# moddyz/stereo-to-multiview-cuda

Measured on AMD Instinct MI355X. Metric: stereo->8-view frames/sec @1080p d=64; cost-agg HBM GB/s vs roofline, higher is better.
Workload: dtype f32; 1 GPU; 1920x1080 synthetic stereo frame, D=64, zd=32, full stereo->8-view frame: cost init + cross aggregation + WTA + DCC/IRV x5/bilateral + 6 DIBR views + interlacing, one frame per GPU per step; stages=3, usd=34, lsd=17, views=8, aggregation=matrix pipe (stm_kernels_aggm.hip)

## Files before the change

stereo-to-multiview-cuda_amd/csrc/stm_common.h:

```cpp
#pragma once
#include <hip/hip_runtime.h>
#include <stddef.h>
#include <stdint.h>

typedef unsigned char u8;

namespace stm {

void fail(const char *what, const char *expr, const char *file, int line);
bool failed();
void clear_failed();
struct ApiNest { ApiNest(); ~ApiNest(); };
bool api_outermost();
void release_host_frame_bufs();
bool nv12_args_ok(const char *fn, int num_rows, int num_cols_sbs, int num_cols, const char *cols_name, int pitch_y, int pitch_uv, int matrix);
#define STM_CHECK(expr)                                                                  \
    do {                                                                                 \
        hipError_t _e = (expr);                                                          \
        if (_e != hipSuccess) ::stm::fail(hipGetErrorString(_e), #expr, __FILE__, __LINE__); \
    } while (0)
#define STM_CHECK_LAUNCH() STM_CHECK(hipGetLastError())
#define STM_LAUNCH(...)                                     \
    do {                                                    \
        if (!::stm::failed()) hipLaunchKernelGGL(__VA_ARGS__); \
// ... 314 lines not shown
bool balance_params_ok(const char *fn, int mode, const u8 *lut768);
bool balance_auto_params_ok(const char *fn, int max_shift, float rate);
bool balance_size_ok(const char *fn, int num_rows, int num_cols);
int balance_rate_q(float rate);
constexpr size_t BALANCE_HIST_WORDS = 1536, BALANCE_STATE_WORDS = 769;
void launch_balance_measure(int *state, uint32_t *hist, const PackInput *in, const u8 *img_l, const u8 *img_r, int H, int W, int elem_sz,
                            int max_shift, int rate_q, bool fresh);
void launch_balance_frame(u8 *out, const PackInput *in, const u8 *img, int H, int W, int elem_sz, const u8 *lut768, const int *state);
struct Cut {
    int mode;
    int thresh_permille, min_gap;
    int *d_state;
};
Cut cut_default();
Cut cut();
void set_cut(const Cut &c);
bool cut_params_ok(const char *fn, int thresh_permille, int min_gap);
bool cut_size_ok(const char *fn, int num_rows, int num_cols);
constexpr size_t CUT_SIG_WORDS = 256, CUT_STATE_WORDS = 260;
constexpr int CUT_DEFAULT_THRESH = 370;
void launch_cut_detect(int *state, uint32_t *sig, const PackInput *in, const u8 *img_l, int H, int W, int elem_sz, int thresh_permille,
                       int min_gap, void *reset0, void *reset1, void *reset2);
struct Active {
    int mode;
    int rect[4];
    int fill;
    float fill_disp;
    int thresh_luma, lit_permille, max_bar_permille, hold;
    int *d_state;
};
Active active_default();
Active active();
void set_active(const Active &a);
bool active_params_ok(const char *fn, int mode, const int *rect, int fill, float fill_disp);
bool active_auto_params_ok(const char *fn, int thresh_luma, int lit_permille, int max_bar_permille, int hold);
bool active_size_ok(const char *fn, int num_rows, int num_cols);
bool active_rect_ok(const char *fn, const int *rect, int num_rows, int num_cols);
constexpr size_t ACTIVE_STATE_WORDS = 16;
void launch_active_detect(int *state, uint32_t *counts, const PackInput *in, const u8 *img_l, int H, int W, int elem_sz, int thresh_luma,
                          int lit_permille, int max_bar_permille, int hold, bool restart, const int *cut_state);
void launch_active_rect(int *d_rect, const int rect[4]);
void launch_active_fill(int nmaps, float *const *disp, int H, int W, const int *d_rect, float value);
struct AggTap {
    float *h1, *v2, *h4;
    const float *inject_v2;
    bool on() const { return h1 || v2 || h4 || inject_v2; }
};
AggTap agg_tap();
void set_agg_tap(const AggTap &t);
enum { TAP_PQ = 0, TAP_PX = 1, TAP_QUADS = 2 };
void launch_tap_read(const float *vol_l, const float *vol_r, int layout, int ord, float *dst, int D, int H, int W);
void launch_tap_write(float *vol_l, float *vol_r, int layout, int ord, const float *src, int D, int H, int W);
struct PQViews {
    const uint32_t *pk[2], *cen[2];
    float *a[2], *b[2];
    const u8 *armU[2], *armD[2], *armL[2], *armR[2];
    float *disp[2];
};
size_t pq_volume_floats(int D, int H, int W);
bool aggm_supports(int usd, int H, int W);
void launch_aggm_frame(const uint32_t *const *pk, const uint32_t *const *cen, const float *lut, float *const *vol_a, float *const *vol_b,
                       const u8 *const *armU, const u8 *const *armD, const u8 *const *armL, const u8 *const *armR, float *const *disp,
                       int D, int zd, int H, int W, int usd, bool keep_volume = false, uint32_t *htab_ready = nullptr, uint32_t *vtab_ready = nullptr,
                       bool v2_read_later = false);
size_t aggm_frame_htab_dwords(int D, int H, int W, int usd, bool keep_volume);
size_t aggm_frame_vtab_dwords(int D, int zd, int H, int W, int usd, bool keep_volume, bool v2_read_later, int *rec, int *top, bool *col);
bool aggm_frame_px(int D, int zd, int H, int W, int usd, bool keep_volume, bool v2_read_later);
int aggm_frame_px_order(int D, int zd, int H, int W, int usd, bool keep_volume, bool v2_read_later);
int aggm_frame_path(int D, int zd, int H, int W, int usd, bool keep_volume, bool v2_read_later);
int aggm_frame_hc2_parts(int D, int zd, int H, int W, int usd, bool keep_volume, bool v2_read_later);
bool launch_aggm_stage(Vol in, Vol out, const u8 *armU, const u8 *armD, const u8 *armL, const u8 *armR, int D, int H, int W, int usd);
size_t aggm_stage_bytes(int D, int H, int W, int usd);
bool aggh_supports(int usd, int D);
size_t aggh_table_dwords(int nviews, int H, int W);
void launch_hwin_table(PQViews &v, int nviews, uint32_t *tab, int H, int W);
void launch_pq_hsr(PQViews &v, int nviews, const uint32_t *tab, int D, int zd, int H, int W, bool px = false, int ord = 0);
bool aggv_supports(int usd);
int aggv_table_top();
int aggv_table_rec();
void launch_pq_v12q(PQViews &v, int nviews, const uint32_t *tab, int rec, int H, int W, int G, int NC);
void launch_pq_v12r(PQViews &v, int nviews, const uint32_t *tab, int H, int W, int G, bool x4 = false);
void launch_vcol_table(PQViews &v, int nviews, uint32_t *tab, int H, int W);
size_t aggv_col_table_dwords(int nviews, int H, int W);
void launch_to_pq(Vol in, float *pq, int D, int H, int W, uint32_t *odd = nullptr);
void launch_from_pq(const float *pq, Vol out, int D, int H, int W);
void launch_hslo_wta(int nviews, const Vol *cost, const u8 *const *img_a, const u8 *const *img_b, const int *osign,
                     float *const *disp, float T, float H1, float H2, int D, int zd, int H, int W, int elem_sz);
void launch_hslo_wta_pq(int nviews, float *const *cost_pq, float *const *acc_pq, const u8 *const *img_a, const u8 *const *img_b,
                        const int *osign, float *const *disp, float T, float H1, float H2, int D, int zd, int H, int W, int elem_sz);

void rho_luts(float ad_coeff, float census_coeff, float *lut_ad , float *lut_census );
void gaussian_kernel_2d(float *kernel, int radius, float sigma);
void gaussian_kernel_1d(float *kernel, int size, float sigma);
float mux_y_interval(int num_views, float angle, int elem_sz);

}
```

stereo-to-multiview-cuda_amd/csrc/stm_hwin.h:

```cpp
#pragma once
#include "stm_common.h"

namespace stm {

constexpr int HR_TOP = 36;
constexpr int HR_NG = 22;
constexpr int HR_REC = 64;

template <int N> __device__ __forceinline__ int hr_row_ror(int v) { return __builtin_amdgcn_update_dpp(0, v, 0x120 + N, 0xf, 0xf, false); }

template <int N> __device__ __forceinline__ uint32_t hr_row_shr(uint32_t v) { return (uint32_t)__builtin_amdgcn_update_dpp(0, (int)v, 0x110 + N, 0xf, 0xf, false); }

static __device__ __forceinline__ void win16_build(uint32_t *__restrict__ dst, uint32_t *ev, int R0, int s0, int nn)
{
    const int m = threadIdx.x & 15;
    int lo = nn ? s0 : 0x7fffffff, hi = nn ? s0 + nn : -0x7fffffff;
    lo = min(lo, hr_row_ror<8>(lo)); lo = min(lo, hr_row_ror<4>(lo)); lo = min(lo, hr_row_ror<2>(lo)); lo = min(lo, hr_row_ror<1>(lo));
    hi = max(hi, hr_row_ror<8>(hi)); hi = max(hi, hr_row_ror<4>(hi)); hi = max(hi, hr_row_ror<2>(hi)); hi = max(hi, hr_row_ror<1>(hi));
    const int K0 = hi > lo ? (lo & ~3) : 0, n = hi > lo ? (hi - K0 + 3) >> 2 : 0;
    const int q0 = n ? (K0 - R0) >> 2 : 0;
#pragma unroll
    for (int i = 0; i < 6; ++i) ev[6 * m + i] = 0u;
    __builtin_amdgcn_wave_barrier();
    if (nn) {
        atomicXor(&ev[s0 - K0], 1u << m);
        atomicXor(&ev[s0 + nn - K0], 1u << m);
    }
    __builtin_amdgcn_wave_barrier();
    uint32_t e[6];
#pragma unroll
    for (int i = 0; i < 6; ++i) e[i] = ev[6 * m + i];
#pragma unroll
    for (int i = 1; i < 6; ++i) e[i] ^= e[i - 1];
    uint32_t tot = e[5];
    tot ^= hr_row_shr<1>(tot); tot ^= hr_row_shr<2>(tot); tot ^= hr_row_shr<4>(tot); tot ^= hr_row_shr<8>(tot);
    const uint32_t before = hr_row_shr<1>(tot);
    __builtin_amdgcn_wave_barrier();
#pragma unroll
    for (int i = 0; i < 6; ++i) ev[6 * m + i] = e[i] ^ before;
    __builtin_amdgcn_wave_barrier();
    if (!dst) return;
    if (m < 2) dst[m] = m == 0 ? (uint32_t)q0 : (uint32_t)n;
#pragma unroll
    for (int j = m; j < HR_NG; j += 16)
        if (j < n) {
            const unsigned long long mk = (unsigned long long)ev[4 * j] | ((unsigned long long)ev[4 * j + 1] << 16) |
                                          ((unsigned long long)ev[4 * j + 2] << 32) | ((unsigned long long)ev[4 * j + 3] << 48);
            *(unsigned long long *)(dst + 8 + 2 * (HR_NG - n + j)) = mk;
        }
}

static __device__ __forceinline__ void hwin_build(uint32_t *__restrict__ tab, uint32_t *ev4, int y, int x0, int aL, int aR, int W, int nTx)
{
    const int l = threadIdx.x & 63, r = l >> 4;
    const int x = x0 + l, t = x >> 4;
    int s0 = 0, nn = 0;
    if (x < W) {
        s0 = x - aL;
        nn = aL + aR;
    }
    win16_build(t < nTx ? tab + ((size_t)y * nTx + t) * HR_REC : nullptr, ev4 + r * 96, 16 * t - HR_TOP, s0, nn);
}

static __device__ __forceinline__ void vcol_build(uint32_t *__restrict__ tile, uint32_t *ev4, int u, int x0, int s0, int nn)
{
    const int r = (threadIdx.x & 63) >> 4;
    win16_build(tile + (size_t)(x0 + r) * HR_REC, ev4 + r * 96, 16 * u - HR_TOP, s0, nn);
}

__device__ __forceinline__ int hw_wave_min_i(int v)
{
    v = min(v, hr_row_ror<8>(v)); v = min(v, hr_row_ror<4>(v)); v = min(v, hr_row_ror<2>(v)); v = min(v, hr_row_ror<1>(v));
    return min(min(__builtin_amdgcn_readlane(v, 0), __builtin_amdgcn_readlane(v, 16)),
               min(__builtin_amdgcn_readlane(v, 32), __builtin_amdgcn_readlane(v, 48)));
}
__device__ __forceinline__ int hw_wave_max_i(int v)
{
    v = max(v, hr_row_ror<8>(v)); v = max(v, hr_row_ror<4>(v)); v = max(v, hr_row_ror<2>(v)); v = max(v, hr_row_ror<1>(v));
    return max(max(__builtin_amdgcn_readlane(v, 0), __builtin_amdgcn_readlane(v, 16)),
               max(__builtin_amdgcn_readlane(v, 32), __builtin_amdgcn_readlane(v, 48)));
}
static __device__ __forceinline__ void vwin_build(uint32_t *__restrict__ dst, unsigned long long *ev, int u, int top, int s0, int nn)
{
    const int l = threadIdx.x & 63;
    const int lo = hw_wave_min_i(nn ? s0 : 0x7fffffff);
    const int hi = hw_wave_max_i(nn ? s0 + nn : -0x7fffffff);
    const int K0 = hi > lo ? (lo & ~3) : 0, n_it = hi > lo ? (hi - K0 + 3) >> 2 : 0;
    const int q0 = top >= 0 && n_it ? (K0 - (16 * u - top)) >> 2 : 0;
    if (l < 8) dst[l] = l == 0 ? (uint32_t)(top >= 0 ? q0 : K0) : l == 1 ? (uint32_t)n_it : 0u;
    unsigned long long *mk = (unsigned long long *)(dst + 8) + 4 * q0;
    const int steps = 4 * n_it;
    for (int j = l; j <= steps; j += 64) ev[j] = 0ull;
    __builtin_amdgcn_wave_barrier();
    if (nn) {
        atomicXor(&ev[s0 - K0], 1ull << l);
        atomicXor(&ev[s0 + nn - K0], 1ull << l);
    }
    __builtin_amdgcn_wave_barrier();
    unsigned long long carry = 0ull;
    for (int base = 0; base < steps; base += 64) {
        unsigned long long e = base + l < steps ? ev[base + l] : 0ull;
#pragma unroll
        for (int o = 1; o < 64; o <<= 1) {
            const unsigned long long t = __shfl_up(e, o);
            if (l >= o) e ^= t;
        }
        e ^= carry;
        if (base + l < steps) mk[base + l] = e;
        carry = __shfl(e, 63);
    }
}

}
```

stereo-to-multiview-cuda_amd/csrc/stm_kernels_agg.hip:

```cpp
#include "stm_hwin.h"

namespace stm {

constexpr uint32_t W10_ONE = 1u | (1u << 10) | (1u << 20);
constexpr uint32_t W10_GUARD = 512u * W10_ONE;

__global__ __launch_bounds__(256) void stm_k_widen_px(const uint32_t *__restrict__ bgrx, uint32_t *__restrict__ wide, int n)
{
    const int i = blockIdx.x * 256 + threadIdx.x;
    if (i >= n) return;
    const uint32_t p = bgrx[i];
    wide[i] = (p & 0xffu) | ((p & 0xff00u) << 2) | ((p & 0xff0000u) << 4);
}


struct ArmsArgs {
    const uint32_t *img[2];
    u8 *up[2], *down[2], *left[2], *right[2];
    uint32_t *htab;
    uint32_t *vtab;
    int vrec, vtop;
    int vcol;
};

// ... 106 lines not shown
        _Pragma("unroll") for (int d = 0; d < 4; ++d)                                                                   \
        {                                                                                                               \
            CT[d] = C[d] + tg_near;                                                                                     \
            const uint32_t ok = (CT[d] - anchor) & (anchor_n - C[d]) & (CT[d] - P[d]) & (PT[d] - C[d]) & W10_GUARD;     \
            STM_ARM_VERDICT(d, ok == W10_GUARD)                                                                         \
        }                                                                                                               \
    }
#define STM_ARM_FAR(K)                                                                     \
    {                                                                                      \
        uint32_t c[4];                                                                     \
        STM_ARM_LOADS(c, K)                                                                \
        _Pragma("unroll") for (int d = 0; d < 4; ++d)                                      \
        {                                                                                  \
            const uint32_t ok = (c[d] + far_lo) & (far_hi - c[d]) & W10_GUARD;             \
            STM_ARM_VERDICT(d, ok == W10_GUARD)                                            \
        }                                                                                  \
    }
    const uint32_t anchor_n = anchor + tg_near;
    uint32_t ca[4], ta[4], cb[4] = {anchor, anchor, anchor, anchor}, tb[4] = {anchor_n, anchor_n, anchor_n, anchor_n};
    const int knear = max(0, min(usd, lsd));
#define STM_ARM_ANY_OPEN (((open[0] | open[1]) | (open[2] | open[3])) != 0ull)
    for (int k = 1; k < knear; k += 2) {
        STM_ARM_CLOSE(k)
        STM_ARM_NEAR(k, ca, ta, cb, tb)
        STM_ARM_NEAR(k + 1, cb, tb, ca, ta)
    }
    if ((knear & 1) && STM_ARM_ANY_OPEN) STM_ARM_NEAR(knear, ca, ta, cb, tb)
    const uint32_t far_lo = tg_far - anchor, far_hi = anchor + tg_far;
    for (int k = knear + 1; k < usd; k += 2) {
        STM_ARM_CLOSE(k)
        STM_ARM_FAR(k)
        STM_ARM_FAR(k + 1)
    }
    if (usd > knear && ((usd - knear) & 1) && STM_ARM_ANY_OPEN) STM_ARM_FAR(usd)
#undef STM_ARM_ANY_OPEN
#undef STM_ARM_FAR
#undef STM_ARM_NEAR
#undef STM_ARM_CLOSE
#undef STM_ARM_VERDICT
#undef STM_ARM_LOADS
    arm[0] = min(arm[0], kmaxU);
    arm[1] = min(arm[1], kmaxD);
    arm[2] = min(arm[2], kmaxL);
    arm[3] = min(arm[3], kmaxR);
}
template <int MODE, bool VMIN>
static __device__ __forceinline__ void cross_arms_body(const ArmsArgs &a, uint32_t tg_far, uint32_t tg_near, int usd, int lsd, int H, int W)
{
    constexpr bool HTAB = MODE >= 1;
    const int v = blockIdx.z;
    const int wv_ = __builtin_amdgcn_readfirstlane((int)(threadIdx.x >> 6));
    const int xr = MODE == 2 ? blockIdx.x * 64 + (threadIdx.x & 63) : blockIdx.x * 256 + threadIdx.x;
    const int yr = MODE == 2 ? blockIdx.y * 16 + wv_ : blockIdx.y;
    if (MODE == 1 ? (xr & ~63) >= W : MODE == 0 ? xr >= W : false) return;
    const int x = min(xr, W - 1), y = min(yr, H - 1);
    const int p = y * W + x;
    int arm[4];
    if (VMIN) cross_arms_walk_vmin(a.img[v], x, y, p, tg_far, tg_near, usd, lsd, H, W, arm);
    else cross_arms_walk(a.img[v], x, y, tg_far, tg_near, usd, lsd, H, W, arm);
    const bool inside = xr < W && yr < H;
    if (inside) {
        a.up[v][p] = (u8)arm[0];
        a.down[v][p] = (u8)arm[1];
        a.left[v][p] = (u8)arm[2];
        a.right[v][p] = (u8)arm[3];
    }
    __shared__ uint32_t ev_all[MODE == 2 ? 16 : 4][4 * 96];
    if (HTAB) {
        const int nTx = (W + 15) >> 4;
        if (yr < H)
            hwin_build(a.htab + (size_t)v * H * nTx * HR_REC, ev_all[wv_], yr, xr & ~63, arm[2], arm[3], W, nTx);
    }
    if (MODE == 2) {
        __shared__ u8 s_u[16][64], s_d[16][64];
        __shared__ unsigned long long ev_v[16][96];
        const int l = threadIdx.x & 63;
        s_u[wv_][l] = inside ? (u8)arm[0] : (u8)0;
        s_d[wv_][l] = inside ? (u8)arm[1] : (u8)0;
        __syncthreads();
        const int G = (W + 3) >> 2, nT = (H + 15) >> 4, gg = blockIdx.x * 16 + wv_, u = blockIdx.y;
        if (gg < G) {
            const int b = l >> 4, i = l & 15;
            const int aU = s_u[i][4 * wv_ + b], aD = s_d[i][4 * wv_ + b];
            if (a.vcol)
                vcol_build(a.vtab + (size_t)(v * nT + u) * (4 * G) * HR_REC, ev_all[wv_], u, 4 * gg, blockIdx.y * 16 + i - aU, aU + aD);
            else
                vwin_build(a.vtab + ((size_t)(v * nT + u) * G + gg) * a.vrec, ev_v[wv_], u, a.vtop, blockIdx.y * 16 + i - aU, aU + aD);
        }
    }
}

template <int MODE>
__global__ __launch_bounds__(MODE == 2 ? 1024 : 256) void stm_k_cross_arms(ArmsArgs a, uint32_t tg_far, uint32_t tg_near, int usd, int lsd, int H, int W)
{
    cross_arms_body<MODE, false>(a, tg_far, tg_near, usd, lsd, H, W);
}

template <int MODE>
__global__ __launch_bounds__(MODE == 2 ? 1024 : 256) void stm_k_cross_arms_vmin(ArmsArgs a, uint32_t tg_far, uint32_t tg_near, int usd, int lsd, int H, int W)
{
    cross_arms_body<MODE, true>(a, tg_far, tg_near, usd, lsd, H, W);
}

static uint32_t wide_threshold(float t)
{
    int ti;
    if (t != t) ti = 255;
    else if (t >= 255.f) ti = 255;
    else if (t < 0.f) ti = -1;
    else ti = (int)floorf(t);
    return (uint32_t)(512 + ti) * W10_ONE;
}

void launch_cross_arms2(int nviews, const uint32_t *const *packed, u8 *const *up, u8 *const *down, u8 *const *left,
                        u8 *const *right, float ucd, float lcd, int usd, int lsd, int H, int W, const uint32_t *const *wide_ready,
                        uint32_t *htab, uint32_t *vtab, int vrec, int vtop, bool vcol)
{
    ArmsArgs a;
    const int n = H * W;
    ProfScope p("cross_arms");
    const uint32_t *wide[2];
    for (int v = 0; v < nviews; ++v) {
        if (wide_ready) {
            wide[v] = wide_ready[v];
            continue;
        }
        uint32_t *w = Workspace::get<uint32_t>((size_t)n);
        STM_LAUNCH(stm_k_widen_px, dim3(cdiv(n, 256)), dim3(256), 0, stream(), packed[v], w, n);
        STM_CHECK_LAUNCH();
        wide[v] = w;
    }
    for (int v = 0; v < 2; ++v) {
        const int s = v < nviews ? v : 0;
        a.img[v] = wide[s]; a.up[v] = up[s]; a.down[v] = down[s]; a.left[v] = left[s]; a.right[v] = right[s];
    }
    if (usd > 255) usd = 255;
    a.htab = htab;
    a.vtab = vtab;
    a.vrec = vrec;
    a.vtop = vtop;
    a.vcol = vcol ? 1 : 0;
    const bool vmin = (agg_variant() / 100) % 10 == 7 || (size_t)H * W * 4 >= ((size_t)1 << 31);
    const uint32_t tg_far = wide_threshold(ucd), tg_near = wide_threshold(lcd);
#define STM_CROSS_LAUNCH(MODE, GRID, BLOCK)                                                                                      \
    {                                                                                                                            \
        if (vmin) STM_LAUNCH(stm_k_cross_arms_vmin<MODE>, GRID, BLOCK, 0, stream(), a, tg_far, tg_near, usd, lsd, H, W);         \
        else STM_LAUNCH(stm_k_cross_arms<MODE>, GRID, BLOCK, 0, stream(), a, tg_far, tg_near, usd, lsd, H, W);                   \
    }
    if (htab && vtab && vtop >= 0 && usd <= HR_TOP && usd <= vtop)
        STM_CROSS_LAUNCH(2, dim3(cdiv(W, 64), cdiv(H, 16), nviews), dim3(1024))
    else if (htab && usd <= HR_TOP)
        STM_CROSS_LAUNCH(1, dim3(cdiv(W, 256), H, nviews), dim3(256))
    else
        STM_CROSS_LAUNCH(0, dim3(cdiv(W, 256), H, nviews), dim3(256))
#undef STM_CROSS_LAUNCH
    STM_CHECK_LAUNCH();
}

void launch_cross_arms(const uint32_t *packed, u8 *up, u8 *down, u8 *left, u8 *right, float ucd, float lcd, int usd,
                       int lsd, int H, int W)
{
    launch_cross_arms2(1, &packed, &up, &down, &left, &right, ucd, lcd, usd, lsd, H, W, nullptr);
}

#define STM_ACC(s, v) { s.x = s.x + v.x; s.y = s.y + v.y; s.z = s.z + v.z; s.w = s.w + v.w; }

template <int S> __device__ __forceinline__ float4 window_sum(const float4 *__restrict__ p, int n, float4 s)
{
    while (n >= 4) {
        float4 v0 = p[0], v1 = p[S], v2 = p[2 * S], v3 = p[3 * S];
        p += 4 * S;
        n -= 4;
        STM_ACC(s, v0) STM_ACC(s, v1) STM_ACC(s, v2) STM_ACC(s, v3)
    }
    if (n & 2) {
        float4 v0 = p[0], v1 = p[S];
        p += 2 * S;
        STM_ACC(s, v0) STM_ACC(s, v1)
    }
    if (n & 1) {
        float4 v0 = p[0];
        STM_ACC(s, v0)
    }
    return s;
}

static void allow_lds(const void *func, size_t bytes)
{
    if (bytes > 64 * 1024) STM_CHECK(hipFuncSetAttribute(func, hipFuncAttributeMaxDynamicSharedMemorySize, (int)bytes));
}

constexpr int AH_QPB = 4;

struct AggHView {
    Vol in, out;
    const u8 *armL, *armR;
    float *disp;
    const uint32_t *pk_own, *cen_own, *pk_oth, *cen_oth;
    int sgn;
};

__device__ __forceinline__ int hamdist_low32(uint32_t a, uint32_t b)
{
    const uint32_t x = a ^ b;
    return __popc(x & 0x7fffffffu) + 33 * (int)(x >> 31);
}

template <bool QUAD, bool WTA, int T, int PPT, bool COST = false>
__global__ __launch_bounds__(T) void stm_k_agg_h(Vol in, Vol out, const u8 *__restrict__ armL,
                                                 const u8 *__restrict__ armR, float *__restrict__ disp,
                                                 int D, int zd, int H, int W, int qpb, AggHView first, AggHView second,
                                                 const float *__restrict__ lut_g)
{
    const AggHView &vw = blockIdx.z ? second : first;
    if (blockIdx.z) {
        in = second.in;
        out = second.out;
        armL = second.armL;
        armR = second.armR;
        disp = second.disp;
    }
    extern __shared__ float4 smem4[];
    float4 *tile = smem4;
    uint16_t *arms = (uint16_t *)(tile + W);
// ... 339 lines not shown
```

stereo-to-multiview-cuda_amd/csrc/stm_kernels_aggv.hip:

```cpp
#include "stm_hwin.h"

namespace stm {

constexpr int VR_TOP = 36;
constexpr int VR_NQ = 22;

template <int EXP>
__global__ __launch_bounds__(64, 2) void stm_k_pq_v12q(PQViews pv, const uint32_t *__restrict__ wtab, int rec, int H, int G, int NC, int nviews)
{
    int wi = blockIdx.x;
    {
        const int per_xcd = gridDim.x >> 3;
        if (wi < 8 * per_xcd) wi = (wi & 7) * per_xcd + (wi >> 3);
    }
    const int c = wi % NC, sidx = wi / NC;
    if (sidx >= G * nviews) return;
    const int g = sidx % G, view = sidx / G;
    const int l = threadIdx.x;
    const int nT = (H + 15) >> 4;
    const int rsb = G * 256;
    const size_t strip = ((size_t)c * H * G + g) * 64;
    const float *in = (const float *)(view ? pv.b[1] : pv.b[0]) + strip;
    float *out = (float *)(view ? pv.a[1] : pv.a[0]) + strip;
    const uint32_t range = (uint32_t)(H - 1) * (uint32_t)rsb + 256u;
// ... 365 lines not shown
        s_cselect_b32 s82, s82, 0             ; first-pass tiles past the image: no window rows (their rows are zeros)
        s_sub_i32 s28, s24, 3
        s_mov_b32 s83, s88
        s_cmp_ge_i32 s28, 0
        s_cselect_b32 s84, s89, 0
        .if VR_EXP & 1
        s_mov_b32 s82, 0
        s_mov_b32 s84, 0
        .endif
        ; headers of the tiles of the step after it (tile indices clamped into the table; unused entries are masked above)
        s_sub_u32 s93, %[nT], 1
        s_add_i32 s92, s24, 1
        s_max_i32 s92, s92, 0
        s_min_i32 s92, s92, s93
        s_mul_i32 s92, s92, %[tstep]
        s_load_dwordx2 s[86:87], %[trow], s92
        s_sub_i32 s92, s24, 2
        s_max_i32 s92, s92, 0
        s_min_i32 s92, s92, s93
        s_mul_i32 s92, s92, %[tstep]
        s_load_dwordx2 s[88:89], %[trow], s92
        s_cmp_eq_u32 s82, 0
        s_cbranch_scc1 VR_noissue1_%=_\@
        s_mov_b32 s94, s81
        s_mov_b32 s95, s82
        s_add_u32 s96, s25, 16                ; row 16 u - 36 = row 16 u + 36 - 72, and -72 = 16 (mod 88)
        s_sub_u32 s31, s96, 88
        s_cmp_ge_u32 s96, 88
        s_cselect_b32 s96, s31, s96
        s_movk_i32 s29, 88
        s_mul_i32 s92, s24, %[tstep]
        s_add_u32 s92, s92, 32
        s_add_u32 s98, %[trow_lo], s92
        s_addc_u32 s99, %[trow_hi], 0
        VR_SWEEP_ISSUE
VR_noissue1_%=_\@:
        VR_STORE_ROWS 0
        VR_STORE_ROWS 1
        VR_STORE_ROWS 2
        VR_STORE_ROWS 3
        .endm
VR_loop_%=:
        VR_STEP 88
        s_cmp_ge_i32 s24, s27
        s_cbranch_scc1 VR_done_%=
        VR_STEP 228
        s_cmp_lt_i32 s24, s27
        s_cbranch_scc1 VR_loop_%=
VR_done_%=:
        s_waitcnt vmcnt(0) lgkmcnt(0)         ; the last rows and headers: nothing may be in flight when the wave ends
        .purgem VR_BLOCK
        .purgem VR_PAIR
        .purgem VR_SWEEP_ISSUE
        .purgem VR_SWEEP_RUN
        .purgem VR_ZERO_ACC
        .purgem VR_PUT4
        .purgem VR_LOAD_ROW
        .purgem VR_LOAD_FAST
        .purgem VR_STORE_ROWS
        .purgem VR_STEP
        )ASM"
                 :
                 : [in] "s"(in), [out] "s"(out), [trow] "s"(trow), [trow_lo] "s"((uint32_t)(uintptr_t)trow), [trow_hi] "s"((uint32_t)((uintptr_t)trow >> 32)),
                   [tstep] "s"(tstep), [rsb] "s"(rsb), [H] "s"(H), [nT] "s"(nT), [range] "s"(range), [voff] "v"(voff), [vst] "v"(vst), [exp] "n"(EXP)
                 : "memory", "scc", "vcc",
                   "s16", "s17", "s18", "s19", "s20", "s21", "s22", "s23", "s24", "s25", "s26", "s27", "s29", "s30", "s31", "s36", "s37", "s38", "s39", "s40", "s41", "s42", "s43", "s44", "s45", "s46", "s47", "s48", "s49", "s50", "s51", "s52", "s53", "s54", "s55", "s56", "s57", "s58", "s59", "s60", "s61", "s62", "s63", "s64", "s65", "s66", "s67", "s68", "s69", "s70", "s71", "s72", "s73", "s74", "s75", "s76", "s77", "s78", "s79", "s80", "s81", "s82", "s83", "s84", "s85", "s86", "s87", "s88", "s89", "s90", "s91", "s92", "s93", "s94", "s95", "s96", "s97", "s98", "s99", "s28",
                   "v0", "v1", "v2", "v3", "v4", "v5", "v6", "v7", "v8", "v9", "v10", "v11", "v12", "v13", "v14", "v15", "v16", "v17", "v18", "v19",
                   "v20", "v21", "v22", "v23", "v24", "v25", "v26", "v27", "v28", "v29", "v30", "v31", "v32", "v33", "v34", "v35", "v36", "v37", "v38", "v39",
                   "v40", "v41", "v42", "v43", "v44", "v45", "v46", "v47", "v48", "v49", "v50", "v51", "v52", "v53", "v54", "v55", "v56", "v57", "v58", "v59",
                   "v60", "v61", "v62", "v63", "v64", "v65", "v66", "v67", "v68", "v69", "v70", "v71", "v72", "v73", "v74", "v75", "v76", "v77", "v78", "v79",
                   "v80", "v81", "v82", "v83", "v84", "v85", "v86", "v87", "v88", "v89", "v90", "v91", "v92", "v93", "v94", "v95", "v96", "v97", "v98", "v99",
                   "v100", "v101", "v102", "v103", "v104", "v105", "v106", "v107", "v108", "v109", "v110", "v111", "v112", "v113", "v114", "v115", "v116",
                   "v117", "v118", "v119", "v120", "v121", "v122", "v123", "v124", "v125", "v126", "v127", "v128", "v129", "v130", "v131", "v132", "v133",
                   "v134", "v135", "v136", "v137", "v138", "v139", "v140", "v141", "v142", "v143", "v144", "v145", "v146", "v147", "v148", "v149", "v150",
                   "v151", "v152", "v153", "v154", "v155", "v156", "v157", "v158", "v159", "v160", "v161", "v162", "v163", "v164", "v165", "v166", "v167",
                   "v168", "v169", "v170", "v171", "v172", "v173", "v174", "v175", "v176", "v177", "v178", "v179", "v180", "v181", "v182", "v183", "v184",
                   "v185", "v186", "v187", "v188", "v189", "v190", "v191", "v192", "v193", "v194", "v195", "v196", "v197", "v198", "v199", "v200", "v201",
                   "v202", "v203", "v204", "v205", "v206", "v207", "v208", "v209", "v210", "v211", "v212", "v213", "v214", "v215", "v216", "v217", "v218",
                   "v219", "v220", "v221", "v222", "v223", "v224", "v225", "v226", "v227", "v228", "v229", "v230", "v231", "v232", "v233", "v234", "v235",
                   "v236", "v237", "v238", "v239", "v240", "v241", "v242", "v243", "v244", "v245", "v246", "v247");
}

template <int EXP, bool X4>
__global__ __launch_bounds__(64, 2) void stm_k_pq_v12r(PQViews pv, const uint32_t *__restrict__ wtab, int H, int G4, int nviews)
{
    const int x = blockIdx.x % G4, view = blockIdx.x / G4;
    if (view >= nviews) return;
    const int l = threadIdx.x;
    const int nT = (H + 15) >> 4;
    const int rsb = G4 * 256;
    const float *in = (const float *)(view ? pv.b[1] : pv.b[0]) + (size_t)x * 64;
    float *out = (float *)(view ? pv.a[1] : pv.a[0]) + (size_t)x * 64;
    const uint32_t range = (uint32_t)(H - 1) * (uint32_t)rsb + 256u;
    const uint32_t *trow = wtab + ((size_t)view * nT * G4 + x) * HR_REC;
    const int tstep = G4 * HR_REC * 4;
    const int voff = 4 * l;
    const int vst = 4 * (l >> 4) * rsb + (l & 15) * (X4 ? 16 : 4);
    asm volatile(R"ASM(
        .set VC_EXP, %[exp]
        .set VC_X4, %[x4]
        ; ---------------------------------------------------------------- macros
        ; one block of a sweep: four MFMAs on one quad of ring rows, the A operand (lanes 16 a + m = row a of the quad, tile row m)
        ; shared through CBSZ / ABID.  p = block index, rb = first register of the ring, acur / anxt = the A registers of this / the
        ; next block
        .macro VC_BLOCK p, rb, acur, anxt
        s_set_gpr_idx_idx s30
        v_mfma_f32_16x16x1_4b_f32 v[204:219], v[\acur], v[\rb], v[204:219] cbsz:2 abid:0
        v_cndmask_b32_e64 v[\anxt], 0, 1.0, s[36+2*((\p)+1):37+2*((\p)+1)]
        v_mfma_f32_16x16x1_4b_f32 v[204:219], v[\acur], v[\rb+1], v[204:219] cbsz:2 abid:1
        s_add_u32 s30, s30, 4
        s_cmp_eq_u32 s30, s29
        s_cselect_b32 s30, 0, s30
        v_mfma_f32_16x16x1_4b_f32 v[204:219], v[\acur], v[\rb+2], v[204:219] cbsz:2 abid:2
        v_mfma_f32_16x16x1_4b_f32 v[204:219], v[\acur], v[\rb+3], v[204:219] cbsz:2 abid:3
        .endm
        .macro VC_PAIR b, rb
        VC_BLOCK 2*(\b), \rb, 220, 221
        VC_BLOCK 2*(\b)+1, \rb, 221, 220
        .endm
        ; the loads a sweep starts from.  q0 / n = the tile's header (n in 1 .. 22), s96 = ring index of the range's first row,
        ; s29 = ring size, s[84:85] = the tile's record.  out: s99 = entry block 22 - n, s30 = ring index of the sweep's first row;
        ; in flight: the 24 mask pairs (block p reads pair p + 1 for its successor, the entry block's own comes through M0)
        .macro VC_SWEEP_ISSUE q0, n
        s_sub_u32 s99, 22, \n
        s_lshl_b32 s31, \q0, 2
        s_add_u32 s30, s96, s31
        s_sub_u32 s31, s30, s29
        s_cmp_ge_u32 s30, s29
        s_cselect_b32 s30, s31, s30
        .if (VC_EXP & 4) == 0
        s_load_dwordx16 s[36:51], s[84:85], 0x20
        s_load_dwordx16 s[52:67], s[84:85], 0x60
        s_load_dwordx16 s[68:83], s[84:85], 0xa0
        .endif
        .endm
        ; the sweep: prologue (the entry block's A operand, first MFMA with the constant 0 as accumulator input), computed jump into
        ; the sequence of blocks, epilogue (the accumulators are read by vector instructions next: the last MFMA must have left
        ; the pipe)
        .macro VC_SWEEP_RUN rb
        s_waitcnt lgkmcnt(0)
        s_lshl_b32 m0, s99, 1
        s_nop 0
        s_movrels_b64 s[86:87], s[36:37]      ; the entry block's mask
        v_cndmask_b32_e64 v220, 0, 1.0, s[86:87]
        v_cndmask_b32_e64 v221, 0, 1.0, s[86:87]
        s_set_gpr_idx_on s30, 0x2
        s_mul_i32 s31, s99, 56
        s_getpc_b64 s[84:85]
VC_pc_%=_\@:
        s_add_u32 s31, s31, VC_blk0_%=_\@-VC_pc_%=_\@+12
        s_add_u32 s84, s84, s31
        s_addc_u32 s85, s85, 0
        v_mfma_f32_16x16x1_4b_f32 v[204:219], v220, v[\rb], 0 cbsz:2 abid:0
        s_setpc_b64 s[84:85]
VC_blk0_%=_\@:
        VC_PAIR 0, \rb
        VC_PAIR 1, \rb
        VC_PAIR 2, \rb
        VC_PAIR 3, \rb
        VC_PAIR 4, \rb
        VC_PAIR 5, \rb
        VC_PAIR 6, \rb
        VC_PAIR 7, \rb
        VC_PAIR 8, \rb
        VC_PAIR 9, \rb
        VC_PAIR 10, \rb
VC_end_%=_\@:
// ... 285 lines not shown
        buffer_store_dwordx4 v[244:247], v224, s[20:23], 0 offen nt
        .endif
        v_mov_b32 v248, v205
        v_mov_b32 v249, v209
        v_mov_b32 v250, v213
        v_mov_b32 v251, v217
        .if (VC_EXP & 2) == 0
        buffer_store_dwordx4 v[248:251], v225, s[20:23], 0 offen nt
        .endif
        v_mov_b32 v244, v206
        v_mov_b32 v245, v210
        v_mov_b32 v246, v214
        v_mov_b32 v247, v218
        .if (VC_EXP & 2) == 0
        buffer_store_dwordx4 v[244:247], v226, s[20:23], 0 offen nt
        .endif
        v_mov_b32 v248, v207
        v_mov_b32 v249, v211
        v_mov_b32 v250, v215
        v_mov_b32 v251, v219
        .if (VC_EXP & 2) == 0
        buffer_store_dwordx4 v[248:251], v227, s[20:23], 0 offen nt
        .endif
        .elseif (VC_EXP & 2) == 0
        buffer_store_dword v204, v224, s[20:23], 0 offen nt
        buffer_store_dword v208, v224, s[20:23], 0 offen offset:64 nt
        buffer_store_dword v212, v224, s[20:23], 0 offen offset:128 nt
        buffer_store_dword v216, v224, s[20:23], 0 offen offset:192 nt
        buffer_store_dword v205, v225, s[20:23], 0 offen nt
        buffer_store_dword v209, v225, s[20:23], 0 offen offset:64 nt
        buffer_store_dword v213, v225, s[20:23], 0 offen offset:128 nt
        buffer_store_dword v217, v225, s[20:23], 0 offen offset:192 nt
        buffer_store_dword v206, v226, s[20:23], 0 offen nt
        buffer_store_dword v210, v226, s[20:23], 0 offen offset:64 nt
        buffer_store_dword v214, v226, s[20:23], 0 offen offset:128 nt
        buffer_store_dword v218, v226, s[20:23], 0 offen offset:192 nt
        buffer_store_dword v207, v227, s[20:23], 0 offen nt
        buffer_store_dword v211, v227, s[20:23], 0 offen offset:64 nt
        buffer_store_dword v215, v227, s[20:23], 0 offen offset:128 nt
        buffer_store_dword v219, v227, s[20:23], 0 offen offset:192 nt
        .endif
        .endm
VC_loop_%=:
        VC_STEP 88
        s_cmp_ge_i32 s24, s27
        s_cbranch_scc1 VC_done_%=
        VC_STEP 228
        s_cmp_lt_i32 s24, s27
        s_cbranch_scc1 VC_loop_%=
VC_done_%=:
        s_waitcnt vmcnt(0) lgkmcnt(0)         ; the last rows, masks and headers: nothing may be in flight when the wave ends
        .purgem VC_BLOCK
        .purgem VC_PAIR
        .purgem VC_SWEEP_ISSUE
        .purgem VC_SWEEP_RUN
        .purgem VC_ZERO_ACC
        .purgem VC_TRANSPOSE
        .purgem VC_PUT4
        .purgem VC_LOAD_ROW
        .purgem VC_LOAD_FAST
        .purgem VC_STEP
        )ASM"
                 :
                 : [in] "s"(in), [out] "s"(out), [trow] "s"(trow), [trow_lo] "s"((uint32_t)(uintptr_t)trow), [trow_hi] "s"((uint32_t)((uintptr_t)trow >> 32)),
                   [tstep] "s"(tstep), [rsb] "s"(rsb), [H] "s"(H), [nT] "s"(nT), [range] "s"(range), [voff] "v"(voff), [vst] "v"(vst), [exp] "n"(EXP), [x4] "n"(X4 ? 1 : 0)
                 : "memory", "scc", "vcc",
                   "s16", "s17", "s18", "s19", "s20", "s21", "s22", "s23", "s24", "s25", "s26", "s27", "s28", "s29", "s30", "s31", "s36", "s37", "s38", "s39", "s40", "s41", "s42", "s43", "s44", "s45", "s46", "s47", "s48", "s49", "s50", "s51", "s52", "s53", "s54", "s55", "s56", "s57", "s58", "s59", "s60", "s61", "s62", "s63", "s64", "s65", "s66", "s67", "s68", "s69", "s70", "s71", "s72", "s73", "s74", "s75", "s76", "s77", "s78", "s79", "s80", "s81", "s82", "s83", "s84", "s85", "s86", "s87", "s88", "s89", "s90", "s91", "s92", "s93", "s94", "s95", "s96", "s97", "s98", "s99",
                   "v0", "v1", "v2", "v3", "v4", "v5", "v6", "v7", "v8", "v9", "v10", "v11", "v12", "v13", "v14", "v15", "v16", "v17", "v18", "v19",
                   "v20", "v21", "v22", "v23", "v24", "v25", "v26", "v27", "v28", "v29", "v30", "v31", "v32", "v33", "v34", "v35", "v36", "v37", "v38", "v39",
                   "v40", "v41", "v42", "v43", "v44", "v45", "v46", "v47", "v48", "v49", "v50", "v51", "v52", "v53", "v54", "v55", "v56", "v57", "v58", "v59",
                   "v60", "v61", "v62", "v63", "v64", "v65", "v66", "v67", "v68", "v69", "v70", "v71", "v72", "v73", "v74", "v75", "v76", "v77", "v78", "v79",
                   "v80", "v81", "v82", "v83", "v84", "v85", "v86", "v87", "v88", "v89", "v90", "v91", "v92", "v93", "v94", "v95", "v96", "v97", "v98", "v99",
                   "v100", "v101", "v102", "v103", "v104", "v105", "v106", "v107", "v108", "v109", "v110", "v111", "v112", "v113", "v114", "v115", "v116",
                   "v117", "v118", "v119", "v120", "v121", "v122", "v123", "v124", "v125", "v126", "v127", "v128", "v129", "v130", "v131", "v132", "v133",
                   "v134", "v135", "v136", "v137", "v138", "v139", "v140", "v141", "v142", "v143", "v144", "v145", "v146", "v147", "v148", "v149", "v150",
                   "v151", "v152", "v153", "v154", "v155", "v156", "v157", "v158", "v159", "v160", "v161", "v162", "v163", "v164", "v165", "v166", "v167",
                   "v168", "v169", "v170", "v171", "v172", "v173", "v174", "v175", "v176", "v177", "v178", "v179", "v180", "v181", "v182", "v183", "v184",
                   "v185", "v186", "v187", "v188", "v189", "v190", "v191", "v192", "v193", "v194", "v195", "v196", "v197", "v198", "v199", "v200", "v201",
                   "v202", "v203", "v204", "v205", "v206", "v207", "v208", "v209", "v210", "v211", "v212", "v213", "v214", "v215", "v216", "v217", "v218",
                   "v219", "v220", "v221", "v224", "v225", "v226", "v227", "v228", "v229", "v230", "v231", "v232", "v233", "v234", "v235",
                   "v236", "v237", "v238", "v239", "v240", "v241", "v242", "v243", "v244", "v245", "v246", "v247", "v248", "v249", "v250", "v251");
}

__global__ __launch_bounds__(256) void stm_k_vcol_table(PQViews v, uint32_t *__restrict__ tab, int H, int W, int G, int nT)
{
    __shared__ uint32_t ev_all[4][4 * 96];
    const int l = threadIdx.x & 63, wv = threadIdx.x >> 6, g = blockIdx.x * 4 + wv, u = blockIdx.y, view = blockIdx.z;
    if (g >= G) return;
    const u8 *__restrict__ armU = view ? v.armU[1] : v.armU[0], *__restrict__ armD = view ? v.armD[1] : v.armD[0];
    const int c = l >> 4, m = l & 15, y = u * 16 + m, x = 4 * g + c;
    int s0 = 0, nn = 0;
    if (y < H && x < W) {
        const int aU = armU[(size_t)y * W + x], aD = armD[(size_t)y * W + x];
        s0 = y - aU;
        nn = aU + aD;
    }
    vcol_build(tab + (size_t)(view * nT + u) * (4 * G) * HR_REC, ev_all[wv], u, 4 * g, s0, nn);
}

bool aggv_supports(int usd) { return usd >= 1 && usd <= VR_TOP; }
int aggv_table_top() { return VR_TOP; }
int aggv_table_rec() { return 8 + 8 * (VR_NQ + 2); }

void launch_pq_v12q(PQViews &v, int nviews, const uint32_t *tab, int rec, int H, int W, int G, int NC)
{
    (void)W;
    const dim3 grid(G * nviews * NC);
#ifdef STM_TIMING
    switch (timing_knobs()) {
    case 1: STM_LAUNCH(stm_k_pq_v12q<1>, grid, dim3(64), 0, stream(), v, tab, rec, H, G, NC, nviews); break;
    case 2: STM_LAUNCH(stm_k_pq_v12q<2>, grid, dim3(64), 0, stream(), v, tab, rec, H, G, NC, nviews); break;
    case 3: STM_LAUNCH(stm_k_pq_v12q<3>, grid, dim3(64), 0, stream(), v, tab, rec, H, G, NC, nviews); break;
    case 4: STM_LAUNCH(stm_k_pq_v12q<4>, grid, dim3(64), 0, stream(), v, tab, rec, H, G, NC, nviews); break;
    case 6: STM_LAUNCH(stm_k_pq_v12q<6>, grid, dim3(64), 0, stream(), v, tab, rec, H, G, NC, nviews); break;
    case 8: STM_LAUNCH(stm_k_pq_v12q<8>, grid, dim3(64), 0, stream(), v, tab, rec, H, G, NC, nviews); break;
    case 9: STM_LAUNCH(stm_k_pq_v12q<9>, grid, dim3(64), 0, stream(), v, tab, rec, H, G, NC, nviews); break;
    default: STM_LAUNCH(stm_k_pq_v12q<0>, grid, dim3(64), 0, stream(), v, tab, rec, H, G, NC, nviews); break;
    }
#else
    STM_LAUNCH(stm_k_pq_v12q<0>, grid, dim3(64), 0, stream(), v, tab, rec, H, G, NC, nviews);
#endif
    STM_CHECK_LAUNCH();
}


size_t aggv_col_table_dwords(int nviews, int H, int W) { return (size_t)nviews * cdiv(H, 16) * (4 * cdiv(W, 4)) * HR_REC + 64; }

void launch_vcol_table(PQViews &v, int nviews, uint32_t *tab, int H, int W)
{
    const int G = cdiv(W, 4), nT = cdiv(H, 16);
    STM_LAUNCH(stm_k_vcol_table, dim3(cdiv(G, 4), nT, nviews), dim3(256), 0, stream(), v, tab, H, W, G, nT);
    STM_CHECK_LAUNCH();
}

void launch_pq_v12r(PQViews &v, int nviews, const uint32_t *tab, int H, int W, int G, bool x4)
{
    (void)W;
    const int G4 = 4 * G;
    const dim3 grid(G4 * nviews);
#define STM_V12R_LAUNCH(E)                                                                                  \
    {                                                                                                       \
        if (x4) STM_LAUNCH((stm_k_pq_v12r<E, true>), grid, dim3(64), 0, stream(), v, tab, H, G4, nviews);   \
        else STM_LAUNCH((stm_k_pq_v12r<E, false>), grid, dim3(64), 0, stream(), v, tab, H, G4, nviews);     \
    }
#ifdef STM_TIMING
    switch (timing_knobs()) {
    case 1: STM_V12R_LAUNCH(1); break;
    case 2: STM_V12R_LAUNCH(2); break;
    case 3: STM_V12R_LAUNCH(3); break;
    case 4: STM_V12R_LAUNCH(4); break;
    case 8: STM_V12R_LAUNCH(8); break;
    default: STM_V12R_LAUNCH(0); break;
    }
#else
    STM_V12R_LAUNCH(0);
#endif
#undef STM_V12R_LAUNCH
    STM_CHECK_LAUNCH();
}

}
```

Baseline: 683.6 frames/s.

## Replace vertical window-mask aggregation with register-ring v_add sequences via computed jumps

Adds a new vertical aggregation kernel that keeps a 72-row ring of input rows and a ring of first-pass sums in VGPRs. For each row it jumps into a precomputed unrolled v_add_f32 sequence whose entry offset encodes the window length, with per-column entry tables built by the column-table kernel. The old mask-table kernel is kept as a variant. It also splits the tail columns into row-range parts to fill the GPU. This is meant to replace the mask/matrix style window evaluation with plain adds and a compact table, at the cost of a large hand-written asm block, clamping windows to 72 rows, and an extra overlap of halo rows per part.

```diff
diff --git a/stereo-to-multiview-cuda_amd/csrc/stm_common.h b/stereo-to-multiview-cuda_amd/csrc/stm_common.h
--- a/stereo-to-multiview-cuda_amd/csrc/stm_common.h
+++ b/stereo-to-multiview-cuda_amd/csrc/stm_common.h
@@ -420,6 +420,7 @@
 void launch_pq_v12r(PQViews &v, int nviews, const uint32_t *tab, int H, int W, int G, bool x4 = false);
 void launch_vcol_table(PQViews &v, int nviews, uint32_t *tab, int H, int W);
 size_t aggv_col_table_dwords(int nviews, int H, int W);
+bool aggv_col_vadd();
 void launch_to_pq(Vol in, float *pq, int D, int H, int W, uint32_t *odd = nullptr);
 void launch_from_pq(const float *pq, Vol out, int D, int H, int W);
 void launch_hslo_wta(int nviews, const Vol *cost, const u8 *const *img_a, const u8 *const *img_b, const int *osign,
diff --git a/stereo-to-multiview-cuda_amd/csrc/stm_hwin.h b/stereo-to-multiview-cuda_amd/csrc/stm_hwin.h
--- a/stereo-to-multiview-cuda_amd/csrc/stm_hwin.h
+++ b/stereo-to-multiview-cuda_amd/csrc/stm_hwin.h
@@ -68,6 +68,19 @@
     win16_build(tile + (size_t)(x0 + r) * HR_REC, ev4 + r * 96, 16 * u - HR_TOP, s0, nn);
 }
 
+constexpr int VA_RING = 72;
+constexpr int VA_LAG = 36;
+constexpr int VA_SEQ = 4 * VA_RING + 4;
+constexpr int VA_PAD = 72;
+static inline __host__ __device__ int va_rows(int H) { return H + 128; }
+static inline __host__ __device__ uint32_t va_entry(int y, int aU, int aD)
+{
+    int L = aU + aD;
+    L = L > VA_RING ? VA_RING : L;
+    const int e = (y + aD - 1 - VA_LAG + 2 * VA_RING) % VA_RING;
+    return (uint32_t)(VA_SEQ * e + 4 * (VA_RING - L));
+}
+
 __device__ __forceinline__ int hw_wave_min_i(int v)
 {
     v = min(v, hr_row_ror<8>(v)); v = min(v, hr_row_ror<4>(v)); v = min(v, hr_row_ror<2>(v)); v = min(v, hr_row_ror<1>(v));
diff --git a/stereo-to-multiview-cuda_amd/csrc/stm_kernels_agg.hip b/stereo-to-multiview-cuda_amd/csrc/stm_kernels_agg.hip
--- a/stereo-to-multiview-cuda_amd/csrc/stm_kernels_agg.hip
+++ b/stereo-to-multiview-cuda_amd/csrc/stm_kernels_agg.hip
@@ -212,7 +212,9 @@
         if (gg < G) {
             const int b = l >> 4, i = l & 15;
             const int aU = s_u[i][4 * wv_ + b], aD = s_d[i][4 * wv_ + b];
-            if (a.vcol)
+            if (a.vcol == 2)
+                a.vtab[((size_t)v * (4 * G) + 4 * gg + b) * va_rows(H) + VA_PAD + blockIdx.y * 16 + i] = va_entry(blockIdx.y * 16 + i, aU, aD);
+            else if (a.vcol)
                 vcol_build(a.vtab + (size_t)(v * nT + u) * (4 * G) * HR_REC, ev_all[wv_], u, 4 * gg, blockIdx.y * 16 + i - aU, aU + aD);
             else
                 vwin_build(a.vtab + ((size_t)(v * nT + u) * G + gg) * a.vrec, ev_v[wv_], u, a.vtop, blockIdx.y * 16 + i - aU, aU + aD);
@@ -269,7 +271,7 @@
     a.vtab = vtab;
     a.vrec = vrec;
     a.vtop = vtop;
-    a.vcol = vcol ? 1 : 0;
+    a.vcol = !vcol ? 0 : aggv_col_vadd() ? 2 : 1;
     const bool vmin = (agg_variant() / 100) % 10 == 7 || (size_t)H * W * 4 >= ((size_t)1 << 31);
     const uint32_t tg_far = wide_threshold(ucd), tg_near = wide_threshold(lcd);
 #define STM_CROSS_LAUNCH(MODE, GRID, BLOCK)                                                                                      \
diff --git a/stereo-to-multiview-cuda_amd/csrc/stm_kernels_aggv.hip b/stereo-to-multiview-cuda_amd/csrc/stm_kernels_aggv.hip
--- a/stereo-to-multiview-cuda_amd/csrc/stm_kernels_aggv.hip
+++ b/stereo-to-multiview-cuda_amd/csrc/stm_kernels_aggv.hip
@@ -471,7 +471,7 @@
 }
 
 template <int EXP, bool X4>
-__global__ __launch_bounds__(64, 2) void stm_k_pq_v12r(PQViews pv, const uint32_t *__restrict__ wtab, int H, int G4, int nviews)
+__global__ __launch_bounds__(64, 2) void stm_k_pq_v12m(PQViews pv, const uint32_t *__restrict__ wtab, int H, int G4, int nviews)
 {
     const int x = blockIdx.x % G4, view = blockIdx.x / G4;
     if (view >= nviews) return;
@@ -923,6 +923,246 @@
                    "v236", "v237", "v238", "v239", "v240", "v241", "v242", "v243", "v244", "v245", "v246", "v247", "v248", "v249", "v250", "v251");
 }
 
+constexpr int V12R_SLOTS = 3 * 4 * 256;
+template <int EXP, bool X4>
+__global__ __launch_bounds__(64) void stm_k_pq_v12r(PQViews pv, const uint32_t *__restrict__ atab, int H, int G4, int nviews, int full, int parts)
+{
+    const int b = blockIdx.x, cidx = b < full ? b : full + (b - full) / parts, part = b < full ? 0 : (b - full) % parts, np = b < full ? 1 : parts;
+    const int x = cidx % G4, view = cidx / G4;
+    if (view >= nviews) return;
+    const int y0 = (int)((long long)H * part / np), y1 = (int)((long long)H * (part + 1) / np);
+    const int ys = max(y0 - 108, -36);
+    const int p1lo = max(y0 - 36, 0), p1n = min(y1 + 36, H) - p1lo;
+    const int l = threadIdx.x;
+    const int rsb = G4 * 256;
+    const float *in = (const float *)(view ? pv.b[1] : pv.b[0]) + (size_t)x * 64;
+    float *out = (float *)(view ? pv.a[1] : pv.a[0]) + (size_t)x * 64;
+    const uint32_t last = (uint32_t)(H - 1) * (uint32_t)rsb, range = last + 256u;
+    const uint32_t *tcol = atab + ((size_t)view * G4 + x) * va_rows(H);
+    const int voff = 4 * l;
+    const int vst = X4 ? 4 * (4 * (l & 15) + (l >> 4)) : 4 * l;
+    static_assert(VA_RING == 72 && VA_LAG == 36 && VA_SEQ == 292 && VA_PAD == 72, "the asm block below is written for these");
+    asm volatile(R"ASM(
+        .set VA_EXP, %[exp]
+        .macro VA_FILL k
+        .if (VA_EXP & 2) == 0
+        buffer_store_dword v0, %[vst], s[20:23], 0 offen nt   ; (empty buffer: counted, not written)
+        buffer_load_dword v[145+\k], %[voff], s[16:19], s26 offen nt
+        .endif
+        s_add_u32 s26, s26, %[rsb]
+        s_min_u32 s26, s26, s27
+        .endm
+        ; one row.  k = step mod 16 (the landing register), cur / nxt = first SGPR of this / the next step's entries, g = 1: either
+        ; pass asks whether its row is one of the block's (the steps at both ends of a range), g = 0: both are (seven scalar
+        ; instructions less)
+        .macro VA_STEP k, cur, nxt, g
+        s_waitcnt lgkmcnt(0)                  ; this step's entries, requested a step ago
+        s_add_u32 s29, s29, 4
+        s_load_dword s[\nxt], s[40:41], s29
+        s_load_dword s[\nxt+1], s[42:43], s29
+        ; ------------------------------------------------------------ second pass of row y - 36
+        .if \g
+        s_sub_u32 s30, s24, s53
+        s_cmp_lt_u32 s30, s54                 ; (unsigned: also false above the range)
+        s_cselect_b32 s22, %[range], 0
+        s_cbranch_scc0 VA_skip2_%=_\@
+        .endif
+        v_mov_b32 v0, 0
+        .if (VA_EXP & 1) == 0
+        s_add_u32 s48, s38, s[\cur+1]
+        s_addc_u32 s49, s39, 0
+        s_swappc_b64 s[50:51], s[48:49]
+        .endif
+VA_skip2_%=_\@:
+        .if (VA_EXP & 2) == 0
+        buffer_store_dword v0, %[vst], s[20:23], s28 offen nt
+        .endif
+        s_add_u32 s28, s28, %[rsb]
+        ; ------------------------------------------------------------ first pass of row y
+        .if \g
+        s_sub_u32 s31, s24, s55
+        s_cmp_lt_u32 s31, s56
+        s_cbranch_scc0 VA_skip1_%=_\@
+        .endif
+        v_mov_b32 v0, 0
+        .if (VA_EXP & 1) == 0
+        s_add_u32 s48, s36, s[\cur]
+        s_addc_u32 s49, s37, 0
+        s_swappc_b64 s[50:51], s[48:49]
+        .endif
+VA_skip1_%=_\@:
+        .if (VA_EXP & 2) == 0
+        s_waitcnt vmcnt(31)                   ; the load of sixteen steps ago (issued since: 15 loads, 16 stores)
+        .endif
+        s_set_gpr_idx_on s25, 0x8
+        v_mov_b32 v73, v0                     ; first-pass row y -> ring 2
+        v_mov_b32 v1, v[145+\k]               ; input row y + 36 -> ring 1
+        s_set_gpr_idx_off
+        .if (VA_EXP & 2) == 0
+        buffer_load_dword v[145+\k], %[voff], s[16:19], s26 offen nt   ; row y + 52 (below the image: the last row again)
+        .endif
+        s_add_u32 s26, s26, %[rsb]
+        s_min_u32 s26, s26, s27
+        s_add_u32 s25, s25, 1
+        s_cmp_eq_u32 s25, 72
+        s_cselect_b32 s25, 0, s25
+        s_add_i32 s24, s24, 1
+        .endm
+
+        ; ---------------------------------------------------------------- setup
+        s_mov_b64 s[16:17], %[in]
+        s_and_b32 s17, s17, 0xffff
+        s_mov_b32 s18, %[range]
+        s_mov_b32 s19, 0x20000
+        s_mov_b64 s[20:21], %[out]
+        s_and_b32 s21, s21, 0xffff
+        s_mov_b32 s22, 0
+        s_mov_b32 s23, 0x20000
+        s_mov_b32 s24, %[ys]                  ; the first steps only bring rows into ring 1 (a column from its top: 36 steps, rows [0, 36))
+        s_mov_b32 s25, %[ys72]
+        s_mov_b32 s27, %[last]
+        s_add_u32 s26, s24, 36
+        s_mul_i32 s26, s26, %[rsb]
+        s_min_u32 s26, s26, s27
+        s_sub_u32 s28, s24, 36
+        s_mul_i32 s28, s28, %[rsb]
+        s_add_u32 s29, s24, 36
+        s_lshl_b32 s29, s29, 2
+        s_mov_b32 s53, %[p2lo]
+        s_mov_b32 s54, %[p2n]
+        s_mov_b32 s55, %[p1lo]
+        s_mov_b32 s56, %[p1n]
+        s_mov_b32 s57, %[mlo]
+        s_mov_b32 s58, %[mhi]
+        s_add_u32 s40, %[tcol_lo], 144
+        s_addc_u32 s41, %[tcol_hi], 0
+        s_mov_b32 s42, %[tcol_lo]
+        s_mov_b32 s43, %[tcol_hi]
+        s_add_u32 s52, %[y1], 36
+        s_load_dword s44, s[40:41], s29
+        s_load_dword s45, s[42:43], s29
+        s_getpc_b64 s[36:37]
+VA_pc_%=:
+        s_add_u32 s36, s36, VA_seq_%=-VA_pc_%=
+        s_addc_u32 s37, s37, 0
+        s_add_u32 s38, s36, 72*292
+        s_addc_u32 s39, s37, 0
+        v_mov_b32 v0, 0
+        VA_FILL 0
+        VA_FILL 1
+        VA_FILL 2
+        VA_FILL 3
+        VA_FILL 4
+        VA_FILL 5
+        VA_FILL 6
+        VA_FILL 7
+        VA_FILL 8
+        VA_FILL 9
+        VA_FILL 10
+        VA_FILL 11
+        VA_FILL 12
+        VA_FILL 13
+        VA_FILL 14
+        VA_FILL 15
+        s_branch VA_loop_%=
+        ; ---------------------------------------------------------------- the sequences: ring 1 (slots e + 1 .. e + 72), then
+        ; ring 2 (its slot of a row lies 36 further on)
+VA_seq_%=:
+        .set VA_e, 0
+        .rept 72
+        .set VA_j, 0
+        .rept 72
+        v_add_f32 v0, v[1+(VA_e+1+VA_j)%%72], v0
+        .set VA_j, VA_j+1
+        .endr
+        s_setpc_b64 s[50:51]
+        .set VA_e, VA_e+1
+        .endr
+        .set VA_e, 0
+        .rept 72
+        .set VA_j, 0
+        .rept 72
+        v_add_f32 v0, v[73+(VA_e+37+VA_j)%%72], v0
+        .set VA_j, VA_j+1
+        .endr
+        s_setpc_b64 s[50:51]
+        .set VA_e, VA_e+1
+        .endr
+VA_seqend_%=:
+        .if (VA_seqend_%=-VA_seq_%=) != 144*292
+        .error "a sequence is not 292 bytes"
+        .endif
+VA_loop_%=:
+        ; sixteen steps that ask (the ends of the range) ...
+        s_cmp_ge_i32 s24, s52
+        s_cbranch_scc1 VA_done_%=
+        VA_STEP 0, 44, 46, 1
+        VA_STEP 1, 46, 44, 1
+        VA_STEP 2, 44, 46, 1
+        VA_STEP 3, 46, 44, 1
+        VA_STEP 4, 44, 46, 1
+        VA_STEP 5, 46, 44, 1
+        VA_STEP 6, 44, 46, 1
+        VA_STEP 7, 46, 44, 1
+        VA_STEP 8, 44, 46, 1
+        VA_STEP 9, 46, 44, 1
+        VA_STEP 10, 44, 46, 1
+        VA_STEP 11, 46, 44, 1
+        VA_STEP 12, 44, 46, 1
+        VA_STEP 13, 46, 44, 1
+        VA_STEP 14, 44, 46, 1
+        VA_STEP 15, 46, 44, 1
+        s_cmp_lt_i32 s24, s57
+        s_cbranch_scc1 VA_loop_%=
+        s_add_u32 s30, s24, 16
+        s_cmp_gt_i32 s30, s58
+        s_cbranch_scc1 VA_loop_%=
+        s_mov_b32 s22, %[range]
+VA_main_%=:
+        ; ... and sixteen that do not, while all sixteen rows belong to both passes
+        VA_STEP 0, 44, 46, 0
+        VA_STEP 1, 46, 44, 0
+        VA_STEP 2, 44, 46, 0
+        VA_STEP 3, 46, 44, 0
+        VA_STEP 4, 44, 46, 0
+        VA_STEP 5, 46, 44, 0
+        VA_STEP 6, 44, 46, 0
+        VA_STEP 7, 46, 44, 0
+        VA_STEP 8, 44, 46, 0
+        VA_STEP 9, 46, 44, 0
+        VA_STEP 10, 44, 46, 0
+        VA_STEP 11, 46, 44, 0
+        VA_STEP 12, 44, 46, 0
+        VA_STEP 13, 46, 44, 0
+        VA_STEP 14, 44, 46, 0
+        VA_STEP 15, 46, 44, 0
+        s_add_u32 s30, s24, 16
+        s_cmp_le_i32 s30, s58
+        s_cbranch_scc1 VA_main_%=
+        s_branch VA_loop_%=
+VA_done_%=:
+        s_waitcnt vmcnt(0) lgkmcnt(0)         ; the last rows and entries: nothing may be in flight when the wave ends
+        .purgem VA_FILL
+        .purgem VA_STEP
+        )ASM"
+                 :
+                 : [in] "s"(in), [out] "s"(out), [tcol_lo] "s"((uint32_t)(uintptr_t)tcol), [tcol_hi] "s"((uint32_t)((uintptr_t)tcol >> 32)), [rsb] "s"(rsb), [y1] "s"(y1),
+                   [ys] "s"(ys), [ys72] "s"((ys + 72) % 72), [p2lo] "s"(36 + y0), [p2n] "s"(y1 - y0), [p1lo] "s"(p1lo), [p1n] "s"(p1n), [mlo] "s"(y0 + 36), [mhi] "s"(min(y1 + 36, H)), [range] "s"(range), [last] "s"(last), [voff] "v"(voff), [vst] "v"(vst), [exp] "n"(EXP)
+                 : "memory", "scc", "vcc",
+                   "s16", "s17", "s18", "s19", "s20", "s21", "s22", "s23", "s24", "s25", "s26", "s27", "s28", "s29", "s30", "s31", "s36", "s37", "s38", "s39", "s40", "s41", "s42", "s43", "s44", "s45", "s46", "s47", "s48", "s49", "s50", "s51", "s52", "s53", "s54", "s55", "s56", "s57", "s58",
+                   "v0", "v1", "v2", "v3", "v4", "v5", "v6", "v7", "v8", "v9", "v10", "v11", "v12", "v13", "v14", "v15", "v16", "v17", "v18", "v19",
+                   "v20", "v21", "v22", "v23", "v24", "v25", "v26", "v27", "v28", "v29", "v30", "v31", "v32", "v33", "v34", "v35", "v36", "v37",
+                   "v38", "v39", "v40", "v41", "v42", "v43", "v44", "v45", "v46", "v47", "v48", "v49", "v50", "v51", "v52", "v53", "v54", "v55",
+                   "v56", "v57", "v58", "v59", "v60", "v61", "v62", "v63", "v64", "v65", "v66", "v67", "v68", "v69", "v70", "v71", "v72", "v73",
+                   "v74", "v75", "v76", "v77", "v78", "v79", "v80", "v81", "v82", "v83", "v84", "v85", "v86", "v87", "v88", "v89", "v90", "v91",
+                   "v92", "v93", "v94", "v95", "v96", "v97", "v98", "v99", "v100", "v101", "v102", "v103", "v104", "v105", "v106", "v107", "v108",
+                   "v109", "v110", "v111", "v112", "v113", "v114", "v115", "v116", "v117", "v118", "v119", "v120", "v121", "v122", "v123", "v124",
+                   "v125", "v126", "v127", "v128", "v129", "v130", "v131", "v132", "v133", "v134", "v135", "v136", "v137", "v138", "v139", "v140",
+                   "v141", "v142", "v143", "v144", "v145", "v146", "v147", "v148", "v149", "v150", "v151", "v152", "v153", "v154", "v155", "v156",
+                   "v157", "v158", "v159", "v160");
+}
+
+template <bool ENTRIES>
 __global__ __launch_bounds__(256) void stm_k_vcol_table(PQViews v, uint32_t *__restrict__ tab, int H, int W, int G, int nT)
 {
     __shared__ uint32_t ev_all[4][4 * 96];
@@ -930,13 +1170,13 @@
     if (g >= G) return;
     const u8 *__restrict__ armU = view ? v.armU[1] : v.armU[0], *__restrict__ armD = view ? v.armD[1] : v.armD[0];
     const int c = l >> 4, m = l & 15, y = u * 16 + m, x = 4 * g + c;
-    int s0 = 0, nn = 0;
+    int aU = 0, aD = 0;
     if (y < H && x < W) {
-        const int aU = armU[(size_t)y * W + x], aD = armD[(size_t)y * W + x];
-        s0 = y - aU;
-        nn = aU + aD;
+        aU = armU[(size_t)y * W + x];
+        aD = armD[(size_t)y * W + x];
     }
-    vcol_build(tab + (size_t)(view * nT + u) * (4 * G) * HR_REC, ev_all[wv], u, 4 * g, s0, nn);
+    if (ENTRIES) tab[((size_t)view * (4 * G) + x) * va_rows(H) + VA_PAD + y] = va_entry(y, aU, aD);
+    else vcol_build(tab + (size_t)(view * nT + u) * (4 * G) * HR_REC, ev_all[wv], u, 4 * g, y - aU, aU + aD);
 }
 
 bool aggv_supports(int usd) { return usd >= 1 && usd <= VR_TOP; }
@@ -965,12 +1205,18 @@
 }
 
 
-size_t aggv_col_table_dwords(int nviews, int H, int W) { return (size_t)nviews * cdiv(H, 16) * (4 * cdiv(W, 4)) * HR_REC + 64; }
+bool aggv_col_vadd() { return (agg_variant() / 100) % 10 != 8; }
+size_t aggv_col_table_dwords(int nviews, int H, int W)
+{
+    if (aggv_col_vadd()) return (size_t)nviews * (4 * cdiv(W, 4)) * va_rows(H) + 64;
+    return (size_t)nviews * cdiv(H, 16) * (4 * cdiv(W, 4)) * HR_REC + 64;
+}
 
 void launch_vcol_table(PQViews &v, int nviews, uint32_t *tab, int H, int W)
 {
     const int G = cdiv(W, 4), nT = cdiv(H, 16);
-    STM_LAUNCH(stm_k_vcol_table, dim3(cdiv(G, 4), nT, nviews), dim3(256), 0, stream(), v, tab, H, W, G, nT);
+    if (aggv_col_vadd()) STM_LAUNCH(stm_k_vcol_table<true>, dim3(cdiv(G, 4), nT, nviews), dim3(256), 0, stream(), v, tab, H, W, G, nT);
+    else STM_LAUNCH(stm_k_vcol_table<false>, dim3(cdiv(G, 4), nT, nviews), dim3(256), 0, stream(), v, tab, H, W, G, nT);
     STM_CHECK_LAUNCH();
 }
 
@@ -979,10 +1225,16 @@
     (void)W;
     const int G4 = 4 * G;
     const dim3 grid(G4 * nviews);
-#define STM_V12R_LAUNCH(E)                                                                                  \
-    {                                                                                                       \
-        if (x4) STM_LAUNCH((stm_k_pq_v12r<E, true>), grid, dim3(64), 0, stream(), v, tab, H, G4, nviews);   \
-        else STM_LAUNCH((stm_k_pq_v12r<E, false>), grid, dim3(64), 0, stream(), v, tab, H, G4, nviews);     \
+    const bool vadd = aggv_col_vadd();
+    const int ncol = G4 * nviews, full = ncol / V12R_SLOTS * V12R_SLOTS, rest = ncol - full;
+    const int parts = rest ? std::max(1, std::min(V12R_SLOTS / rest, H / 128)) : 1;
+    const dim3 grid_a(full + rest * parts);
+#define STM_V12R_LAUNCH(E)                                                                                      \
+    {                                                                                                           \
+        if (vadd && x4) STM_LAUNCH((stm_k_pq_v12r<E, true>), grid_a, dim3(64), 0, stream(), v, tab, H, G4, nviews, full, parts);   \
+        else if (vadd) STM_LAUNCH((stm_k_pq_v12r<E, false>), grid_a, dim3(64), 0, stream(), v, tab, H, G4, nviews, full, parts);   \
+        else if (x4) STM_LAUNCH((stm_k_pq_v12m<E, true>), grid, dim3(64), 0, stream(), v, tab, H, G4, nviews);      \
+        else STM_LAUNCH((stm_k_pq_v12m<E, false>), grid, dim3(64), 0, stream(), v, tab, H, G4, nviews);             \
     }
 #ifdef STM_TIMING
     switch (timing_knobs()) {
```

Measured after the change: 703.2 frames/s, median of 6. +2.9%, better.
